# WangSimiao2000/MinecraftSkin_Raytracer

Measured on AMD Instinct MI355X. Metric: Mpixels/s, higher is better.
Workload: dtype f32; 1 GPU; 1920x1080, 4 bounces, 4 spp, 1 light, synthetic 64x64 skin (S64), pose 0, soft shadows 8, tile 32; parallelism=single GPU, frames_in_flight=4, hw_queues=4

## Files before the change

### include/mcrt.h

```cpp
#ifndef MCRT_H
#define MCRT_H

#include <stddef.h>
#include <stdint.h>

#ifdef __cplusplus
extern "C" {
#endif

#define MCRT_ABI_VERSION 3

#define MCRT_OK 0
#define MCRT_ERR_INVALID 1
#define MCRT_ERR_NO_DEVICE 2
#define MCRT_ERR_HIP 3
#define MCRT_ERR_NOMEM 4

typedef struct mcrt_config {
    int32_t width;
    int32_t height;
    int32_t max_bounces;
    int32_t samples_per_pixel;
    int32_t tile_size;
    int32_t thread_count;
// ... 308 lines not shown
int mcrt_build_skin_scene_model(const uint8_t* skin_rgba8, int skin_width, int skin_height, int model,
                                const float pose[12], mcrt_scene_desc** out);
int mcrt_scene_create_skin_model(int skin_height, int model, const float pose[12], const mcrt_scene_desc* look, int device, mcrt_scene** out);
int mcrt_skin_texel_model(int skin_height, int model, int mesh, int face_slot, int tx, int ty, int* skin_x, int* skin_y);
int mcrt_skin_pool_map_model(int skin_height, int model, int32_t* out, int capacity);
int mcrt_skin_view_table_model(int skin_height, int model, const float pose[12], const mcrt_scene_desc* look, void* out, size_t capacity);
int mcrt_skin_model_of(const uint8_t* skin_rgba8, int skin_width, int skin_height);
int mcrt_build_default_scene(const float pose[12], mcrt_scene_desc** out);
int mcrt_builtin_pose(int index, float pose_out[12]);
void mcrt_scene_desc_free(mcrt_scene_desc* desc);

size_t mcrt_scene_flatten(const mcrt_scene_desc* desc, void* blob, size_t capacity);

typedef struct mcrt_hit {
    int32_t hit;
    float t;
    float point[3];
    float normal[3];
    float texture_color[4];
    int32_t is_outer_layer;
} mcrt_hit;

int mcrt_probe_scene_blob(mcrt_scene* scene, void* out, size_t capacity);
int mcrt_probe_intersect(mcrt_scene* scene, const float* rays, int n, mcrt_hit* out);
int mcrt_probe_trace(mcrt_scene* scene, const mcrt_config* cfg, const float* rays, int n, int depth,
                     float* out_rgba);
int mcrt_probe_mt_uniform(int device, const uint32_t* seeds, int n_seeds, int n_draws, float* out);
int mcrt_probe_detmath(int device, int op, const float* x, const float* y, size_t n, float* out);
int mcrt_probe_detmath_range(int device, int op, uint32_t lo_bits, uint32_t hi_bits, float y0,
                             uint64_t* mismatches);
int mcrt_probe_div_const(int device, uint32_t d_first, uint32_t d_count, int mode, uint64_t* mismatches, uint32_t* a_failing_divisor);

#ifdef __cplusplus
}
#endif
#endif
```

### minecraftskin_raytracer_amd/_lib.py

```python
from __future__ import annotations

import ctypes as C
import os

from . import abi

PKG = os.path.dirname(os.path.abspath(__file__))
LIB_PATH = os.environ.get("MCRT_LIB") or os.path.join(PKG, "libmcrt.so")

_lib = None

EXPORTED_SYMBOLS = [
    "mcrt_config_init", "mcrt_generate_tiles", "mcrt_abi_version", "mcrt_device_count", "mcrt_last_error",
    "mcrt_render", "mcrt_render_tile", "mcrt_scene_create", "mcrt_scene_destroy", "mcrt_render_device", "mcrt_owned_pixel_rows",
    "mcrt_unpack_rows_device", "mcrt_quantize_rgba8_device", "mcrt_quantize_rgba8", "mcrt_last_timings",
    "mcrt_time_render_device", "mcrt_build_skin_scene", "mcrt_build_default_scene", "mcrt_builtin_pose",
    "mcrt_scene_desc_free", "mcrt_scene_flatten", "mcrt_probe_intersect", "mcrt_probe_trace",
    "mcrt_probe_mt_uniform", "mcrt_probe_detmath", "mcrt_probe_detmath_range", "mcrt_probe_div_const",
    "mcrt_render_device_ex", "mcrt_write_png_rgba8", "mcrt_encode_png_rgba8", "mcrt_write_png_f32", "mcrt_render_png",
    "mcrt_assemble_frame_device", "mcrt_scene_set_lanes", "mcrt_trim", "mcrt_scene_check", "mcrt_render_multi",
    "mcrt_render_rgba8", "mcrt_render_rect", "mcrt_render_batch_device", "mcrt_render_batch", "mcrt_last_batch_info",
    "mcrt_scene_set_background", "mcrt_render_ex", "mcrt_render_batch_ex", "mcrt_render_png_ex",
    "mcrt_bg_plate_info", "mcrt_draw_plate_info",
    "mcrt_render_layers_device", "mcrt_render_layers_batch_device", "mcrt_render_layers", "mcrt_render_layers_batch",
    "mcrt_scene_pick", "mcrt_skin_texel",
    "mcrt_render_ground_device", "mcrt_render_ground_batch_device", "mcrt_render_ground", "mcrt_scene_floor",
    "mcrt_render_reflection_device", "mcrt_render_reflection_batch_device", "mcrt_render_reflection",
    "mcrt_render_light_device", "mcrt_render_light_batch_device", "mcrt_render_light",
    "mcrt_scene_create_skin", "mcrt_scene_set_skin_device", "mcrt_scene_set_skins_batch_device", "mcrt_scene_set_skin",
    "mcrt_skin_pool_map", "mcrt_probe_scene_blob",
    "mcrt_bake_light_device", "mcrt_bake_light_batch_device", "mcrt_bake_light", "mcrt_bake_texel_table", "mcrt_scene_texels",
    "mcrt_scene_set_view", "mcrt_scene_set_view_device", "mcrt_scene_set_views_batch_device", "mcrt_skin_view_table",
    "mcrt_shot_init", "mcrt_shot_scratch_bytes", "mcrt_composite_shot_batch_device", "mcrt_render_shot_batch_device",
    "mcrt_render_shot_device", "mcrt_render_shot", "mcrt_render_shot_batch", "mcrt_render_shot_png",
    "mcrt_render_ground_occlusion_device", "mcrt_render_ground_occlusion_batch_device", "mcrt_render_ground_occlusion",
    "mcrt_shot_scratch_bytes_occ", "mcrt_render_shot_batch_device_occ", "mcrt_composite_shot_batch_device_occ",
    "mcrt_render_shot_batch_occ", "mcrt_render_shot_png_occ",
    "mcrt_shot_ex_init", "mcrt_shot_scratch_bytes_ex", "mcrt_composite_shot_batch_device_ex", "mcrt_render_shot_batch_device_ex",
    "mcrt_render_shot_batch_ex", "mcrt_render_shot_png_ex",
    "mcrt_build_skin_scene_model", "mcrt_scene_create_skin_model", "mcrt_skin_texel_model", "mcrt_skin_pool_map_model",
    "mcrt_skin_view_table_model", "mcrt_skin_model_of",
]


def load():
    global _lib
    if _lib is not None:
        return _lib
    if not os.path.exists(LIB_PATH):
        raise RuntimeError(
            f"{LIB_PATH} is missing: build it with `python -m minecraftskin_raytracer_amd.build` "
            "(hipcc --offload-arch=gfx950). There is no CPU fallback."
        )
# ... 141 lines not shown
```

### minecraftskin_raytracer_amd/api.py

```python
from __future__ import annotations

import ctypes as C
import os
from typing import Callable, List, Optional, Sequence, Tuple

import numpy as np

from . import abi
from ._lib import McrtError, check, load
from .abi import Config, Mesh, Scene, SceneDescHolder, Texture

Image = np.ndarray


def trim() -> None:
    load().mcrt_trim()


def device_count() -> int:
    return int(load().mcrt_device_count())


class _OwnedDescPtr(C.POINTER(abi.McrtSceneDesc)):

# ... 599 lines not shown
        self._skin_bytes()
        check(load().mcrt_scene_set_skin_device(self._h, C.c_void_p(ptr or None), C.c_void_p(stream)))

    def set_view(self, pose: Optional[Sequence[float]] = None, look=None) -> None:
        self._skin_bytes()
        p, d = _view_pose(pose), _as_desc(look) if look is not None else None
        check(load().mcrt_scene_set_view(self._h, abi.fptr(p) if p is not None else None, d.ptr if d is not None else None))

    def set_view_device(self, pose: Optional[Sequence[float]] = None, look=None, stream: int = 0) -> None:
        self._skin_bytes()
        p, d = _view_pose(pose), _as_desc(look) if look is not None else None
        check(load().mcrt_scene_set_view_device(self._h, abi.fptr(p) if p is not None else None, d.ptr if d is not None else None, C.c_void_p(stream)))

    def blob(self) -> bytes:
        lib = load()
        head = C.create_string_buffer(192)
        n = lib.mcrt_probe_scene_blob(self._h, head, 192)
        if n < 192:
            raise McrtError(n, lib.mcrt_last_error().decode("utf-8", "replace"))
        buf = C.create_string_buffer(n)
        if lib.mcrt_probe_scene_blob(self._h, buf, n) != n:
            raise McrtError(abi.MCRT_ERR_HIP, lib.mcrt_last_error().decode("utf-8", "replace"))
        return buf.raw

    def close(self):
        if self._h:
            load().mcrt_scene_destroy(self._h)
            self._h = C.c_void_p()

    def __del__(self):
        try:
            self.close()
        except Exception:
            pass

    def check(self) -> None:
        check(load().mcrt_scene_check(self._h))

    def set_lanes(self, lanes: int) -> None:
        check(load().mcrt_scene_set_lanes(self._h, int(lanes)))

    def set_background(self, mode: str) -> None:
        m = abi.background_mode(mode)
        check(load().mcrt_scene_set_background(self._h, m))

    def owned_pixel_rows(self, config: Config, first: int = 0, step: int = 1) -> int:
# ... 525 lines not shown
```

### minecraftskin_raytracer_amd/csrc/kernel_common.h

```cpp
#ifndef MCRT_KERNEL_COMMON_H
#define MCRT_KERNEL_COMMON_H

#include "kernels.h"
#include "rt_core.h"

#include <type_traits>

#ifdef MCRT_KERNEL_HOOKS
#include MCRT_KERNEL_HOOKS
#else
#define MCRT_HOOK_LIT_SHARED
#define MCRT_HOOK_LIT_CLASSIFIED(known, undecided, cand, O)
#define MCRT_HOOK_LIT_SHADED(lit, r)
#define MCRT_HOOK_RESOLVE_BEGIN()
#endif

namespace mcrt {

using namespace rt;

struct UDiv {
    unsigned d;
    int shift;
    __device__ __forceinline__ explicit UDiv(unsigned dv) : d(dv), shift((dv & (dv - 1u)) == 0u && dv != 0u ? static_cast<int>(__builtin_ctz(dv)) : -1) {}
    __device__ __forceinline__ unsigned div(unsigned n) const { return shift >= 0 ? n >> shift : n / d; }
};

struct TileGeom {
    int x, y, w, h;
    int owned_row;
    int frame_tile;
};

__device__ __forceinline__ uchar4 quantize_pixel(float4 c) {
    uchar4 q;
    q.x = static_cast<unsigned char>(sclamp(c.x, 0.0f, 1.0f) * 255.0f + 0.5f);
    q.y = static_cast<unsigned char>(sclamp(c.y, 0.0f, 1.0f) * 255.0f + 0.5f);
    q.z = static_cast<unsigned char>(sclamp(c.z, 0.0f, 1.0f) * 255.0f + 0.5f);
    q.w = static_cast<unsigned char>(sclamp(c.w, 0.0f, 1.0f) * 255.0f + 0.5f);
    return q;
}

__device__ __forceinline__ bool mesh_touches_tile(const FlatMesh& m, const TileGeom& t, const mcrt_config& cfg,
                                                  float aspect, float lens_pad) {
    float u0 = m.screen[0], v0 = m.screen[1], u1 = m.screen[2], v1 = m.screen[3];
    if (u0 > u1) return true;
    u0 -= lens_pad, v0 -= lens_pad, u1 += lens_pad, v1 += lens_pad;
    const float W = static_cast<float>(cfg.width), H = static_cast<float>(cfg.height);
    float tu0 = (2.0f * (static_cast<float>(t.x) - 2.0f) / W - 1.0f) * aspect - 1e-3f * aspect - 1e-3f;
    float tu1 = (2.0f * (static_cast<float>(t.x + t.w) + 2.0f) / W - 1.0f) * aspect + 1e-3f * aspect + 1e-3f;
    float tv1 = 1.0f - 2.0f * (static_cast<float>(t.y) - 2.0f) / H + 2e-3f;
    float tv0 = 1.0f - 2.0f * (static_cast<float>(t.y + t.h) + 2.0f) / H - 2e-3f;
    return !(u1 < tu0 || u0 > tu1 || v1 < tv0 || v0 > tv1);
}

struct LdsTables {
// ... 230 lines not shown
```

### minecraftskin_raytracer_amd/csrc/kernels.h

```cpp
#ifndef MCRT_KERNELS_H
#define MCRT_KERNELS_H

#include <hip/hip_runtime.h>
#include <stdint.h>

#include <vector>

#include "launch_shapes.h"
#include "mcrt.h"

namespace mcrt {

struct Shard {
    int first;
    int step;
    int tiles_x;
    int tiles_y;
    int owned_rows;
    int pack_first;
    int pack_step;
};

struct WaveSpace {
    float4* scol;
// ... 27 lines not shown
constexpr int kDivFrameMax = 16384;

constexpr uint32_t kSeedWindowHalf = 1u << 24;
constexpr uint32_t kSeedWindow = 1u << 25;

struct RenderParams {
    const uint8_t* scene;
    const uint32_t* seed_table;
    const uint32_t* seed_table_full;
    mcrt_config cfg;
    Shard shard;
    int layout;
    float* out;
    uint8_t* out8;
    uint32_t* tile_rng;
    const float4* bg_plate;
    const float* draw_plate;
    WaveSpace ws;
    int draws_per_sample;
    int stream_waves;
    int stream_parts;
    int stream_part_twists;
    int parts_per_tile;
    int lds_alpha_words;
    int lds_face_entries;
    int scene_in_lds;
    int scene_posed;
    int rows_per_batch;
    int bg_in_plan;
    int bg_kernel;
    int background;
    int lit_round;
    int lit_pass;
    int lit_lds_offset;
    int lit_lds_bytes;
    int flat;
    float inv_width, inv_height;
    int div_frame;
    int inside_fast;
    int bundle_decisions;
    int work_tickets;
    int shared_device;
    int grid_primary, grid_ao, grid_lit, grid_resolve;
    int rect_x, rect_y, rect_w, rect_h;
};

// ... 309 lines not shown
```

### minecraftskin_raytracer_amd/csrc/probes.cpp

```cpp
#include "host_internal.h"
#include "mcrt_detmath.h"

#include <cmath>
#include <thread>

using namespace mcrt;
using namespace mcrt_host;

namespace {
int finish_probe(hipError_t launched, void* out, const DeviceBuffer& d_out, size_t bytes, const char* what) {
    hipError_t e = launched;
    if (e == hipSuccess) e = hipMemcpy(out, d_out.ptr, bytes, hipMemcpyDeviceToHost);
    if (e != hipSuccess) return hip_fail(e, what);
    return MCRT_OK;
}
}

extern "C" {

int mcrt_probe_intersect(mcrt_scene* s, const float* rays, int n, mcrt_hit* out) {
    if (!s || !rays || !out || n < 0) return fail(MCRT_ERR_INVALID, "bad argument");
    if (n == 0) return MCRT_OK;
    HIP_TRY(hipSetDevice(s->device));
    DeviceBuffer d_rays, d_out;
    HIP_TRY(d_rays.reserve(static_cast<size_t>(n) * 24));
    HIP_TRY(d_out.reserve(static_cast<size_t>(n) * sizeof(mcrt_hit)));
    HIP_TRY(hipMemcpy(d_rays.ptr, rays, static_cast<size_t>(n) * 24, hipMemcpyHostToDevice));
    hipError_t e = launch_probe_intersect(static_cast<const uint8_t*>(s->blob.ptr), static_cast<float*>(d_rays.ptr), n,
                                          static_cast<mcrt_hit*>(d_out.ptr), nullptr);
    return finish_probe(e, out, d_out, static_cast<size_t>(n) * sizeof(mcrt_hit), "probe_intersect");
}

int mcrt_probe_scene_blob(mcrt_scene* s, void* out, size_t capacity) {
    if (!s || !out) return fail(MCRT_ERR_INVALID, "NULL argument");
    HIP_TRY(hipSetDevice(s->device));
    HIP_TRY(hipDeviceSynchronize());
    if (s->host_meshes.size() < sizeof(FlatHeader) || !s->blob.ptr) return fail(MCRT_ERR_INVALID, "the handle holds no scene");
    const size_t bytes = reinterpret_cast<const FlatHeader*>(s->host_meshes.data())->blob_bytes;
    HIP_TRY(hipMemcpy(out, s->blob.ptr, bytes < capacity ? bytes : capacity, hipMemcpyDeviceToHost));
    return static_cast<int>(bytes);
}

int mcrt_probe_trace(mcrt_scene* s, const mcrt_config* cfg, const float* rays, int n, int depth, float* out_rgba) {
    if (!s || !cfg || !rays || !out_rgba || n < 0) return fail(MCRT_ERR_INVALID, "bad argument");
    if (n == 0) return MCRT_OK;
    HIP_TRY(hipSetDevice(s->device));
    DeviceBuffer d_rays, d_out, d_rng, d_stack;
    HIP_TRY(d_rays.reserve(static_cast<size_t>(n) * 24));
    HIP_TRY(d_out.reserve(static_cast<size_t>(n) * 16));
    bool long_rng = (cfg->soft_shadows && 2 * cfg->shadow_samples > 227) || (cfg->ao_enabled && 2 * cfg->ao_samples > 227);
    if (long_rng) HIP_TRY(d_rng.reserve(static_cast<size_t>(n) * 624 * 4));
    if (cfg->max_bounces > 16) HIP_TRY(d_stack.reserve(static_cast<size_t>(n) * cfg->max_bounces * 16));
    HIP_TRY(hipMemcpy(d_rays.ptr, rays, static_cast<size_t>(n) * 24, hipMemcpyHostToDevice));
    hipError_t e = launch_probe_trace(static_cast<const uint8_t*>(s->blob.ptr), *cfg, static_cast<float*>(d_rays.ptr), n,
                                      depth, static_cast<float*>(d_out.ptr), static_cast<uint32_t*>(d_rng.ptr),
                                      static_cast<float*>(d_stack.ptr), nullptr);
    return finish_probe(e, out_rgba, d_out, static_cast<size_t>(n) * 16, "probe_trace");
}

int mcrt_probe_mt_uniform(int device, const uint32_t* seeds, int n_seeds, int n_draws, float* out) {
    if (!seeds || !out || n_seeds < 0 || n_draws < 0) return fail(MCRT_ERR_INVALID, "bad argument");
    if (n_seeds == 0 || n_draws == 0) return MCRT_OK;
    if (mcrt_device_count() <= 0) return fail(MCRT_ERR_NO_DEVICE, "no HIP device");
// ... 97 lines not shown
```

### minecraftskin_raytracer_amd/csrc/render_enqueue.cpp

```cpp
#include "host_internal.h"

#include <algorithm>
#include <cmath>
#include <cstring>

using namespace mcrt;
using namespace mcrt_host;

namespace {

thread_local int t_background_override = -1;
struct BackgroundOverride {
    explicit BackgroundOverride(int mode) { t_background_override = mode; }
    ~BackgroundOverride() { t_background_override = -1; }
    BackgroundOverride(const BackgroundOverride&) = delete;
    BackgroundOverride& operator=(const BackgroundOverride&) = delete;
};

int draws_per_sample(const mcrt_config& c) {
    int spp = c.samples_per_pixel > 1 ? c.samples_per_pixel : 1;
    return (spp > 1 ? 2 : 0) + ((c.dof_enabled && c.aperture > 1e-6f) ? 2 : 0);
}

int lane_count(const mcrt_scene* s, const mcrt_config& cfg, const Shard& sh) {
// ... 58 lines not shown
            for (int tx = tx0; tx <= tx1; ++tx) grid[static_cast<size_t>(ty) * sh.tiles_x + tx] = 1;
    }
    for (int j = 0; j < sh.owned_rows; ++j) {
        const int ty = sh.first + j * sh.step;
        int c = 0;
        for (int tx = 0; tx < sh.tiles_x; ++tx) c += grid[static_cast<size_t>(ty) * sh.tiles_x + tx];
        out[static_cast<size_t>(j)] = c;
    }
}

int prepare(mcrt_scene* sc, int li, int n_lanes, const mcrt_config* cfg, int first, int step, int layout, float* d_out,
            uint8_t* d_out8, RenderParams& p, std::vector<int>* row_touched_out = nullptr, const mcrt_tile* rect = nullptr) {
    Lane* s = &sc->lanes[li];
    std::memset(&p, 0, sizeof p);
    p.scene = static_cast<const uint8_t*>(sc->blob.ptr);
    p.seed_table = sc->seed_table;
    p.seed_table_full = sc->seed_table_full;
    static const bool decisions = !env_off("MCRT_BUNDLE_DECISIONS");
    p.bundle_decisions = decisions ? 1 : 0;
    static const bool inside_fast = !env_off("MCRT_INSIDE_FAST");
    p.inside_fast = inside_fast ? 1 : 0;
    static const bool work_tickets = !env_off("MCRT_WORK_TICKETS");
    p.work_tickets = work_tickets ? 1 : 0;
    p.cfg = *cfg;
    if (cfg->width > 0 && cfg->height > 0) {
        p.inv_width = 1.0f / static_cast<float>(cfg->width);
        p.inv_height = 1.0f / static_cast<float>(cfg->height);
        static const bool fast_div = !env_off("MCRT_DIV_FRAME");
        p.div_frame = (fast_div && cfg->width <= kDivFrameMax && cfg->height <= kDivFrameMax) ? 1 : 0;
    }
    p.shard = make_shard(*cfg, first + li * step, step * n_lanes);
    p.shard.pack_first = li;
    p.shard.pack_step = n_lanes;
    if (rect) {
        p.rect_x = rect->x, p.rect_y = rect->y, p.rect_w = rect->width, p.rect_h = rect->height;
        p.shard.first = 0, p.shard.step = 1, p.shard.tiles_x = 1, p.shard.tiles_y = 1, p.shard.owned_rows = 1;
        p.shard.pack_first = 0, p.shard.pack_step = 1;
    }
    p.layout = layout;
    p.out = d_out;
    p.out8 = d_out8;
    p.background = rect ? MCRT_BACKGROUND_REFERENCE : (t_background_override >= 0 ? t_background_override : sc->background);
    p.draws_per_sample = draws_per_sample(*cfg);
    const LdsFit fit = lds_fit(sc->alpha_words, sc->n_meshes, sc->posed);
    p.scene_in_lds = fit.view != kViewHbm ? 1 : 0;
    p.scene_posed = sc->posed ? 1 : 0;
// ... 1237 lines not shown
```

### minecraftskin_raytracer_amd/csrc/render_kernels.hip

```cpp
#include "kernel_common.h"

namespace mcrt {

using namespace rt;

struct FrameDiv {
    float w, h, rw, rh;
    bool fast;
    __device__ __forceinline__ explicit FrameDiv(const RenderParams& p)
        : w(static_cast<float>(p.cfg.width)), h(static_cast<float>(p.cfg.height)), rw(p.inv_width), rh(p.inv_height), fast(p.div_frame != 0) {}
    __device__ __forceinline__ float u(float x) const { return fast ? div_frame(x, w, rw) : x / w; }
    __device__ __forceinline__ float v(float y) const { return fast ? div_frame(y, h, rh) : y / h; }
};

__device__ __forceinline__ TileGeom tile_of(const RenderParams& p, int owned_tile) {
    TileGeom t;
    if (p.rect_w > 0) {
        t.x = p.rect_x, t.y = p.rect_y, t.w = p.rect_w, t.h = p.rect_h;
        t.owned_row = 0;
        t.frame_tile = 0;
        return t;
    }
    int k = owned_tile / p.shard.tiles_x;
    int tx = owned_tile - k * p.shard.tiles_x;
// ... 289 lines not shown
        const FlatMesh& m = sc.meshes[lane];
        float lens_pad = 0.0f;
        if (dof) {
            const float half_h = sc.hdr->cam_half_h, half_w = half_h * aspect;
            const float focus = cfg.focus_distance > 0.0f ? cfg.focus_distance : sc.hdr->cam_focus_auto;
            const float inv_f_lo = 1.0f / focus;
            const float inv_f_hi = __builtin_sqrtf(1.0f + half_w * half_w + half_h * half_h) / focus;
            const float inv_z_hi = 1.0f / m.depth[0], inv_z_lo = 1.0f / m.depth[1];
            const float d = fmaxf(fmaxf(fabsf(inv_z_hi - inv_f_lo), fabsf(inv_z_hi - inv_f_hi)),
                                  fmaxf(fabsf(inv_z_lo - inv_f_lo), fabsf(inv_z_lo - inv_f_hi)));
            lens_pad = cfg.aperture * d / half_h * 1.02f + 1e-3f;
            const float err = 4.0f * 1.1920929e-7f * (sc.hdr->mask_slack * (1.0f / kMaskSlack) + focus + cfg.aperture);
            const float r2 = half_w * half_w + half_h * half_h;
            const float rel = err * inv_f_hi * (1.0f + __builtin_sqrtf(r2));
            lens_pad += (2.0f * rel + err * inv_z_hi) / half_h;
            if (!(m.depth[0] > 0.0f) || !(focus > 0.0f) || !(lens_pad < 1e6f) || !(rel < 0.05f)) lens_pad = 1e30f;
        }
        touch = mesh_touches_tile(m, tg, cfg, aspect, lens_pad);
    }
    unsigned long long mask = __ballot(touch);
    if (!cull && sc.n_meshes > 0) mask = ~0ull;
    return mask;
}
__device__ __forceinline__ uint32_t plan_touched_tile(const RenderParams& p, const TileGeom& tg, int tile, unsigned long long mask) {
    const mcrt_config& cfg = p.cfg;
    const WaveSpace& ws = p.ws;
    ws.tile_mask[tile] = mask;
    if (mask == 0ull) return ~0u;
    const uint32_t spp = cfg.samples_per_pixel > 1 ? cfg.samples_per_pixel : 1;
    const uint32_t npix = static_cast<uint32_t>(tg.w) * static_cast<uint32_t>(tg.h);
    const uint32_t parts = static_cast<uint32_t>(p.parts_per_tile);
    const uint32_t per = (npix + parts - 1u) / parts;
    const uint32_t used = (npix + per - 1u) / per;
    const uint32_t ord = count_add(ws, kCntTiles, 1u);
    if (ord >= ws.tile_cap) {
        ws.counters[kCntOverflow] = 1u;
        ws.tile_mask[tile] = 0ull;
        return ~0u;
    }
    const uint32_t slot0 = count_add(ws, kCntUnits, used);
    const uint32_t base = ord * ws.tile_slots;
    for (uint32_t i = 0; i < used; ++i) {
        const uint32_t a = i * per, b = min(npix, a + per);
        ws.units[slot0 + i] = make_uint4(static_cast<uint32_t>(tile), a, b, base + a * spp);
    }
    return ord;
}

__device__ __forceinline__ void plan_tiles_body(const uint8_t* __restrict__ scene_blob, const uint32_t* __restrict__ tile_rng,
                                                float* __restrict__ tile_draws, float4* __restrict__ out_frame, uchar4* __restrict__ out8,
                                                const RenderParams& __restrict__ p, const int tile_base, const int n_tiles) {
    __shared__ __align__(16) uint32_t s_state[kStreamWaves][2 * 624];
    __shared__ uint32_t s_ord[kStreamWaves];
    const int wave = threadIdx.x >> 6, lane = threadIdx.x & 63;
    const int parts = p.stream_waves;
    const int per_wave = p.stream_parts / parts;
    const int slot = static_cast<int>(blockIdx.x) * kStreamWaves + wave;
    const int t = slot / parts, part = slot - t * parts;
    const bool valid = t < n_tiles;
    const int tile = tile_base + (valid ? t : 0);
    const TileGeom tg = tile_of(p, tile);
    const SceneView sc = view_of(scene_blob);
    const unsigned long long mask = valid ? tile_mesh_mask(sc, p, tg, lane) : 0ull;
    if (valid && part == 0 && lane == 0) s_ord[wave] = plan_touched_tile(p, tg, tile, mask);
    if (parts > 1) {
        __syncthreads();
    } else {
        __builtin_amdgcn_fence(__ATOMIC_SEQ_CST, "wavefront");
        __builtin_amdgcn_wave_barrier();
    }
    if (!valid) return;
    const uint32_t ord = s_ord[wave - part];
    const size_t stride = p.ws.draws_stride;
    const unsigned npix = static_cast<unsigned>(tg.w) * static_cast<unsigned>(tg.h);
    if (!p.bg_in_plan) {
        float4 unused;
        if (p.draws_per_sample > 0 && !(mask == 0ull && constant_background(sc, p, tg, unused)))
            tile_stream_wave(sc, tile_rng, tile_draws + static_cast<size_t>(t) * stride, nullptr, nullptr, p, tg, tile, part * per_wave, per_wave, s_state[wave], lane,
                             mask == 0ull && p.draws_per_sample == 4);
    } else if (mask != 0ull) {
        if (p.draws_per_sample > 0 && ord != ~0u && !p.draw_plate)
            tile_stream_wave(sc, tile_rng, tile_draws + static_cast<size_t>(ord) * stride, nullptr, nullptr, p, tg, tile, part * per_wave, per_wave, s_state[wave], lane);
    } else if (p.background == MCRT_BACKGROUND_TRANSPARENT) {
        fill_tile(p, tg, out_frame, out8, make_float4(0.0f, 0.0f, 0.0f, 0.0f), static_cast<unsigned>(part * 64 + lane), static_cast<unsigned>(parts) * 64u);
    } else if (float4 pixel; constant_background(sc, p, tg, pixel)) {
        fill_tile(p, tg, out_frame, out8, pixel, static_cast<unsigned>(part * 64 + lane), static_cast<unsigned>(parts) * 64u);
    } else if (p.cfg.samples_per_pixel > 1) {
// ... 100 lines not shown

    const SceneView scg = view_of(scene_blob);
    const mcrt_config& cfg = p.cfg;
    const WaveSpace& ws = p.ws;
    const uint32_t n_units = counted(ws, kCntUnits);
    if (blockIdx.x == 0 && threadIdx.x == 0) ws.frame_info[0] = n_units;
    if ((p.bg_in_plan || p.bg_kernel) && blockIdx.x >= n_units) return;
    const bool bounce_here = p.flat && cfg.max_bounces >= 1;
    const bool posed = kView != kViewLdsUnposed && p.scene_posed != 0;
    const typename ViewSel<kView>::type sc = ViewSel<kView>::make(scg, p, s_dyn);
    const int tid = threadIdx.x;
    const int spp = cfg.samples_per_pixel > 1 ? cfg.samples_per_pixel : 1;
    const int dd = p.draws_per_sample;
    const bool dof = cfg.dof_enabled && cfg.aperture > 1e-6f;
    const float aspect = static_cast<float>(cfg.width) / static_cast<float>(cfg.height);
    const FrameDiv fd(p);
    float focusDist = cfg.focus_distance;
    if (focusDist <= 0.0f) focusDist = sc.hdr->cam_focus_auto;
    const size_t stride = ws.draws_stride;

    uint32_t turn = 0;
    for (uint32_t u = blockIdx.x; u < n_units; u = next_work(p, kCntTicketPrimary, u, n_units, s_ticket, turn)) {
        const uint4 ud = ws.units[u];
        const int tile = static_cast<int>(ud.x);
        const unsigned pp0 = ud.y, pp1 = ud.z;
        const uint32_t slot_base = ud.w;
        const TileGeom tg = tile_of(p, tile);
        const unsigned long long mesh_mask = ws.tile_mask[tile];
        const float* draws = tile_draws + static_cast<size_t>(p.draw_plate ? static_cast<uint32_t>(tg.frame_tile)
                                                              : p.bg_in_plan ? slot_base / ws.tile_slots : static_cast<uint32_t>(tile - tile_base)) * stride;
        const unsigned n_samples = (pp1 - pp0) * static_cast<unsigned>(spp);

        uint32_t unit_hits = 0;
        for (unsigned s0 = 0; s0 < n_samples; s0 += kChunk) {
            bool is_hit = false;
            Ray ray{mk(0, 0, 0), mk(0, 0, 0)};
            Hit hit;
            hit.hit = false;
            uint32_t sample_slot = 0;
            const unsigned sidx = s0 + tid;
            if (sidx < n_samples) {
                const unsigned pix = pp0 + UDiv(static_cast<unsigned>(spp)).div(sidx);
                const unsigned uly = UDiv(static_cast<unsigned>(tg.w)).div(pix);
                const int ly = static_cast<int>(uly);
                const int lx = static_cast<int>(pix - uly * static_cast<unsigned>(tg.w));
                const int px = tg.x + lx, py = tg.y + ly;
                const float* jd = draws + (static_cast<size_t>(pp0) * spp + sidx) * dd;
                float jx = 0.5f, jy = 0.5f;
                int dpos = 0;
                if (spp > 1) {
                    jx = jd[0];
                    jy = jd[1];
                    dpos = 2;
                }
                const float su = fd.u(static_cast<float>(px) + jx);
                const float sv = fd.v(static_cast<float>(py) + jy);
                sample_slot = slot_base + sidx;
                ray = dof ? lens_ray(sc, su, sv, aspect, cfg.aperture, focusDist, jd[dpos], jd[dpos + 1])
                          : camera_ray(sc, su, sv, aspect);
                hit = hit_scene(sc, ray, mesh_mask);
                uint32_t code = kEndMiss;
                if (hit.hit && cfg.max_bounces < 0) {
                    const C4 col = background(sc, cfg, 0.5f, 0.5f);
                    ws.scol[sample_slot] = make_float4(col.r, col.g, col.b, col.a);
                    code = 0u;
                } else if (hit.hit) {
                    is_hit = true;
                    code = (p.flat && cfg.max_bounces == 0) ? 3u : 0u;
                }
                ws.end[sample_slot] = code;
// ... 753 lines not shown
        --dd;
    }
    for (; dd >= 0; --dd) {
        const float4 sd = lv[dd * plane];
        tail = fold_reflection(C4{sd.x, sd.y, sd.z, sd.w}, tail);
    }
    return make_float4(tail.r, tail.g, tail.b, tail.a);
}
template <bool kTransparent>
__device__ __forceinline__ void resolve_body(const uint8_t* __restrict__ scene_blob, const float* __restrict__ tile_draws,
                                             float4* __restrict__ out_frame, uchar4* __restrict__ out8, const RenderParams& __restrict__ p,
                                             const int tile_base) {
    __shared__ ResolveLds<kTransparent> s_lds;
    float4* s_col = s_lds.col;
    const WaveSpace& ws = p.ws;
    const mcrt_config& cfg = p.cfg;
    const SceneView scg = view_of(scene_blob);
    const FrameDiv fd(p);
    const uint32_t dd = static_cast<uint32_t>(p.draws_per_sample);
    auto unit_sample = [&](const uint4& d, const TileGeom& tg, const float* draws, uint32_t sidx, uint32_t spp_) __attribute__((always_inline)) -> float4 {
        const uint32_t slot = d.w + sidx;
        const uint32_t code = ws.end[slot];
        if (code != kEndMiss) return sample_colour(ws, slot, code, C4{scg.hdr->background[0], scg.hdr->background[1], scg.hdr->background[2], scg.hdr->background[3]});
        const unsigned pix = d.y + UDiv(spp_).div(sidx);
        const unsigned uly = UDiv(static_cast<unsigned>(tg.w)).div(pix);
        const int px = tg.x + static_cast<int>(pix - uly * static_cast<unsigned>(tg.w)), py = tg.y + static_cast<int>(uly);
        float jx = 0.5f, jy = 0.5f;
        if (spp_ > 1u) {
            const float2 j = *reinterpret_cast<const float2*>(draws + (static_cast<size_t>(d.y) * spp_ + sidx) * dd);
            jx = j.x, jy = j.y;
        }
        const C4 c = background(scg, cfg, fd.u(static_cast<float>(px) + jx), fd.v(static_cast<float>(py) + jy));
        return make_float4(c.r, c.g, c.b, c.a);
    };
    const uint32_t n_units = ws.frame_info[0];
    const uint32_t spp = cfg.samples_per_pixel > 1 ? static_cast<uint32_t>(cfg.samples_per_pixel) : 1u;
    const float inv_spp = 1.0f / static_cast<float>(spp);
    const uint32_t chunk_px = spp <= static_cast<uint32_t>(kBlock) ? static_cast<uint32_t>(kBlock) / spp : 0u;
    auto put_pixel = [&](const TileGeom& tg, uint32_t i, float4 acc) __attribute__((always_inline)) {
        const uint32_t uly = i / static_cast<uint32_t>(tg.w);
        const int ly = static_cast<int>(uly);
        const int lx = static_cast<int>(i - uly * static_cast<uint32_t>(tg.w));
        const int row = (p.layout == MCRT_LAYOUT_PACKED) ? ((p.shard.pack_first + tg.owned_row * p.shard.pack_step) * cfg.tile_size + ly) : (tg.y + ly);
        store_pixel(out_frame, out8, static_cast<size_t>(row) * cfg.width + (tg.x + lx),
                    make_float4(acc.x * inv_spp, acc.y * inv_spp, acc.z * inv_spp, acc.w * inv_spp));
    };
    auto hit_sample = [&](const uint4& d, uint32_t sidx, bool& hit) __attribute__((always_inline)) -> float4 {
        const uint32_t slot = d.w + sidx;
        const uint32_t code = ws.end[slot];
        hit = code != kEndMiss;
        if (!hit) return make_float4(0.0f, 0.0f, 0.0f, 0.0f);
        return sample_colour(ws, slot, code, C4{scg.hdr->background[0], scg.hdr->background[1], scg.hdr->background[2], scg.hdr->background[3]});
    };
    auto put_pixel_transparent = [&](const TileGeom& tg, uint32_t i, float4 acc, uint32_t n) __attribute__((always_inline)) {
        float4 v = make_float4(0.0f, 0.0f, 0.0f, 0.0f);
        if (n > 0u) {
            const float inv_n = 1.0f / static_cast<float>(n);
            v = make_float4(acc.x * inv_n, acc.y * inv_n, acc.z * inv_n, acc.w * inv_spp);
        }
        const uint32_t uly = i / static_cast<uint32_t>(tg.w);
        const int ly = static_cast<int>(uly);
        const int lx = static_cast<int>(i - uly * static_cast<uint32_t>(tg.w));
        const int row = (p.layout == MCRT_LAYOUT_PACKED) ? ((p.shard.pack_first + tg.owned_row * p.shard.pack_step) * cfg.tile_size + ly) : (tg.y + ly);
        store_pixel(out_frame, out8, static_cast<size_t>(row) * cfg.width + (tg.x + lx), v);
    };
    MCRT_HOOK_RESOLVE_BEGIN()
    if (blockIdx.x == 0) {
        for (int i = threadIdx.x; i < kCounterWords - 4; i += kBlock) ws.counter_base[i] = ws.counters[i];
    }
    for (uint32_t u = blockIdx.x; u < n_units; u += gridDim.x) {
        const uint4 d = ws.units[u];
        const TileGeom tg = tile_of(p, static_cast<int>(d.x));
        const uint32_t pp0 = d.y, pp1 = d.z;
        const float* draws = tile_draws + static_cast<size_t>(p.draw_plate ? static_cast<uint32_t>(tg.frame_tile)
                                                              : p.bg_in_plan ? d.w / ws.tile_slots : static_cast<uint32_t>(static_cast<int>(d.x) - tile_base)) * ws.draws_stride;
        if (chunk_px == 0u) {
            for (uint32_t i = pp0 + threadIdx.x; i < pp1; i += kBlock) {
                float4 acc = make_float4(0.0f, 0.0f, 0.0f, 0.0f);
                if constexpr (kTransparent) {
                    uint32_t n = 0;
                    for (uint32_t s = 0; s < spp; ++s) {
                        bool hit;
                        const float4 c = hit_sample(d, (i - pp0) * spp + s, hit);
                        if (!hit) continue;
                        acc.x += c.x, acc.y += c.y, acc.z += c.z, acc.w += c.w;
                        ++n;
                    }
                    put_pixel_transparent(tg, i, acc, n);
                } else {
                    for (uint32_t s = 0; s < spp; ++s) {
                        const float4 c = unit_sample(d, tg, draws, (i - pp0) * spp + s, spp);
                        acc.x += c.x, acc.y += c.y, acc.z += c.z, acc.w += c.w;
                    }
                    put_pixel(tg, i, acc);
                }
            }
            continue;
        }
        for (uint32_t p0 = pp0; p0 < pp1; p0 += chunk_px) {
            const uint32_t npx = min(chunk_px, pp1 - p0);
            if constexpr (kTransparent) {
                if (threadIdx.x < npx * spp) {
                    bool hit;
                    s_col[threadIdx.x] = hit_sample(d, (p0 - pp0) * spp + threadIdx.x, hit);
                    s_lds.hit[threadIdx.x] = hit ? 1 : 0;
                }
            } else {
                if (threadIdx.x < npx * spp) s_col[threadIdx.x] = unit_sample(d, tg, draws, (p0 - pp0) * spp + threadIdx.x, spp);
            }
            __syncthreads();
            if (threadIdx.x < npx) {
                float4 acc = make_float4(0.0f, 0.0f, 0.0f, 0.0f);
                if constexpr (kTransparent) {
                    uint32_t n = 0;
                    for (uint32_t s = 0; s < spp; ++s) {
                        if (!s_lds.hit[threadIdx.x * spp + s]) continue;
                        const float4 c = s_col[threadIdx.x * spp + s];
                        acc.x += c.x, acc.y += c.y, acc.z += c.z, acc.w += c.w;
                        ++n;
                    }
                    put_pixel_transparent(tg, p0 + threadIdx.x, acc, n);
                } else {
                    for (uint32_t s = 0; s < spp; ++s) {
                        const float4 c = s_col[threadIdx.x * spp + s];
                        acc.x += c.x, acc.y += c.y, acc.z += c.z, acc.w += c.w;
                    }
                    put_pixel(tg, p0 + threadIdx.x, acc);
                }
            }
            __syncthreads();
        }
    }
}
__global__ __launch_bounds__(kBlock) void resolve_kernel(const uint8_t* __restrict__ scene_blob, const float* __restrict__ tile_draws,
                                                         float4* __restrict__ out_frame, uchar4* __restrict__ out8, const RenderParams p,
                                                         const int tile_base) {
    resolve_body<false>(scene_blob, tile_draws, out_frame, out8, p, tile_base);
}
__global__ __launch_bounds__(kBlock) void resolve_transparent_kernel(const uint8_t* __restrict__ scene_blob, float4* __restrict__ out_frame,
                                                                     uchar4* __restrict__ out8, const RenderParams p, const int tile_base) {
    resolve_body<true>(scene_blob, nullptr, out_frame, out8, p, tile_base);
}

using ParamTable = const __attribute__((address_space(4))) RenderParams*;
__device__ __forceinline__ const RenderParams& frame_params(ParamTable table) { return *(const RenderParams*)(table + blockIdx.y); }
__global__ __launch_bounds__(64) void seed_tiles_batch_kernel(ParamTable table, int n_tiles) {
    seed_tiles_body(frame_params(table), n_tiles);
}
__global__ __launch_bounds__(64 * kStreamWaves) void advance_tiles_batch_kernel(ParamTable table, int n_tiles) {
    advance_tiles_body(frame_params(table), n_tiles);
// ... 168 lines not shown
```

### minecraftskin_raytracer_amd/csrc/render_plan.cpp

```cpp
#include "kernels.h"

#include "flat_scene.h"

#include <algorithm>
#include <cstdlib>
#include <cstring>

namespace mcrt {

using rt::kMtShortMax;

Shard make_shard(const mcrt_config& cfg, int first, int step) {
    Shard s{};
    s.first = first;
    s.step = step < 1 ? 1 : step;
    s.pack_first = 0;
    s.pack_step = 1;
    if (cfg.width <= 0 || cfg.height <= 0 || cfg.tile_size <= 0) return s;
    s.tiles_x = (cfg.width + cfg.tile_size - 1) / cfg.tile_size;
    s.tiles_y = (cfg.height + cfg.tile_size - 1) / cfg.tile_size;
    s.owned_rows = (first < s.tiles_y && first >= 0) ? (s.tiles_y - first + s.step - 1) / s.step : 0;
    return s;
}

static int int_knob(const char* name, int fallback) {
    const char* e = getenv(name);
    const int v = e ? atoi(e) : 0;
    return v > 0 ? v : fallback;
}

static bool needs_general_variant(const mcrt_config& c) {
    return (c.ao_enabled && (c.ao_samples <= 0 || 2 * c.ao_samples > kMtShortMax)) || (soft_sampling(c) && 2 * c.shadow_samples > kMtShortMax) ||
           c.max_bounces > kFlatMaxBounces;
}

static int choose_parts_per_tile(const RenderParams& p) {
    const mcrt_config& cfg = p.cfg;
    const long long spp = cfg.samples_per_pixel > 1 ? cfg.samples_per_pixel : 1;
    const long long tile_items = p.rect_w > 0 ? static_cast<long long>(p.rect_w) * p.rect_h * spp : static_cast<long long>(cfg.tile_size) * cfg.tile_size * spp;
    long long parts = (tile_items + kChunk - 1) / kChunk;
    const long long most = p.rect_w > 0 ? 4096 : 16;
    if (parts > most) parts = most;
    if (parts < 1) parts = 1;
    return static_cast<int>(parts);
}

WorkspaceBytes plan_workspace(RenderParams& p, size_t budget_bytes, const int* row_touched) {
    WorkspaceBytes w{};
    const mcrt_config& c = p.cfg;
    const int n_tiles = owned_tiles(p);
    p.parts_per_tile = choose_parts_per_tile(p);
    p.flat = needs_general_variant(c) ? 0 : 1;
    p.ws.stack_stride = c.max_bounces > 0 ? c.max_bounces + 1 : 1;
    const size_t spp = c.samples_per_pixel > 1 ? c.samples_per_pixel : 1;
    const size_t tile_w = p.rect_w > 0 ? static_cast<size_t>(p.rect_w) : static_cast<size_t>(c.tile_size < c.width ? c.tile_size : c.width);
    const size_t tile_h = p.rect_w > 0 ? static_cast<size_t>(p.rect_h) : static_cast<size_t>(c.tile_size < c.height ? c.tile_size : c.height);
    const size_t tile_slots = tile_w * tile_h * spp;
    const size_t S = soft_sampling(c) ? static_cast<size_t>(c.shadow_samples) : 0;
    const size_t A = c.ao_enabled && c.ao_samples > 0 ? static_cast<size_t>(c.ao_samples) : 0;
    const size_t rays = S > A ? S : A;
    const size_t recs = p.flat ? static_cast<size_t>(1 + (c.max_bounces > 0 ? c.max_bounces : 0)) : 2;
    const size_t hbm_rays = p.flat ? 0 : rays;
    const size_t ray_recs = p.flat ? 1 : recs;
    const size_t per_entry = 16 + 4 + recs * (5 * 16 + 4) + ray_recs * (12 * hbm_rays + (hbm_rays ? 8 : 0) + 4) + 4 + 16 * static_cast<size_t>(p.ws.stack_stride);
    {
        const size_t pairs = S ? S : 1;
        size_t pass = kLitLdsBytes / (12 * pairs);
// ... 308 lines not shown
```

Measured before the change: 19450 Mpixels/s.

## Split tiles into compact 2D pixel blocks instead of row-range units

Work units inside a tile can now be rectangular sub-blocks (chosen near-square, fitting one chunk) instead of contiguous row ranges. Compact blocks should make rays within a unit more coherent, which helps cache reuse and cuts divergence in traversal. Unit emission in the planner is also spread across wave lanes instead of lane 0 only. The cost is an extra pixel mapping (a divide plus an offset) per sample and a new unit encoding that the primary and resolve kernels must share. A probe API for inspecting unit records is added as well.

```diff
diff --git a/include/mcrt.h b/include/mcrt.h
--- a/include/mcrt.h
+++ b/include/mcrt.h
@@ -354,6 +354,7 @@
 } mcrt_hit;
 
 int mcrt_probe_scene_blob(mcrt_scene* scene, void* out, size_t capacity);
+int mcrt_probe_units(mcrt_scene* scene, uint32_t* records, uint32_t* hits, int capacity);
 int mcrt_probe_intersect(mcrt_scene* scene, const float* rays, int n, mcrt_hit* out);
 int mcrt_probe_trace(mcrt_scene* scene, const mcrt_config* cfg, const float* rays, int n, int depth,
                      float* out_rgba);
diff --git a/minecraftskin_raytracer_amd/_lib.py b/minecraftskin_raytracer_amd/_lib.py
--- a/minecraftskin_raytracer_amd/_lib.py
+++ b/minecraftskin_raytracer_amd/_lib.py
@@ -28,7 +28,7 @@
     "mcrt_render_reflection_device", "mcrt_render_reflection_batch_device", "mcrt_render_reflection",
     "mcrt_render_light_device", "mcrt_render_light_batch_device", "mcrt_render_light",
     "mcrt_scene_create_skin", "mcrt_scene_set_skin_device", "mcrt_scene_set_skins_batch_device", "mcrt_scene_set_skin",
-    "mcrt_skin_pool_map", "mcrt_probe_scene_blob",
+    "mcrt_skin_pool_map", "mcrt_probe_scene_blob", "mcrt_probe_units",
     "mcrt_bake_light_device", "mcrt_bake_light_batch_device", "mcrt_bake_light", "mcrt_bake_texel_table", "mcrt_scene_texels",
     "mcrt_scene_set_view", "mcrt_scene_set_view_device", "mcrt_scene_set_views_batch_device", "mcrt_skin_view_table",
     "mcrt_shot_init", "mcrt_shot_scratch_bytes", "mcrt_composite_shot_batch_device", "mcrt_render_shot_batch_device",
diff --git a/minecraftskin_raytracer_amd/api.py b/minecraftskin_raytracer_amd/api.py
--- a/minecraftskin_raytracer_amd/api.py
+++ b/minecraftskin_raytracer_amd/api.py
@@ -645,6 +645,17 @@
         if lib.mcrt_probe_scene_blob(self._h, buf, n) != n:
             raise McrtError(abi.MCRT_ERR_HIP, lib.mcrt_last_error().decode("utf-8", "replace"))
         return buf.raw
+
+    def units(self) -> dict:
+        fn = load().mcrt_probe_units
+        fn.restype, fn.argtypes = C.c_int, [C.c_void_p, C.c_void_p, C.c_void_p, C.c_int]
+        n = fn(self._h, None, None, 0)
+        if n < 0:
+            raise McrtError(n, load().mcrt_last_error().decode("utf-8", "replace"))
+        rec, hits = np.zeros((n, 4), np.uint32), np.zeros(n, np.uint32)
+        if n and fn(self._h, rec.ctypes.data, hits.ctypes.data, n) != n:
+            raise McrtError(abi.MCRT_ERR_HIP, load().mcrt_last_error().decode("utf-8", "replace"))
+        return {"records": rec, "hits": hits}
 
     def close(self):
         if self._h:
diff --git a/minecraftskin_raytracer_amd/csrc/kernel_common.h b/minecraftskin_raytracer_amd/csrc/kernel_common.h
--- a/minecraftskin_raytracer_amd/csrc/kernel_common.h
+++ b/minecraftskin_raytracer_amd/csrc/kernel_common.h
@@ -32,6 +32,28 @@
     int frame_tile;
 };
 
+constexpr uint32_t kUnitBlock = 1u << 31;
+__device__ __forceinline__ int unit_tile(const uint4& ud) { return static_cast<int>(ud.x & ~kUnitBlock); }
+__device__ __forceinline__ uint32_t unit_pixels(const uint4& ud) { return (ud.x & kUnitBlock) ? (ud.z & 0xffffu) * (ud.z >> 16) : ud.z - ud.y; }
+struct UnitMap {
+    uint32_t koff, x0, y0;
+    UDiv by_w;
+    __device__ __forceinline__ UnitMap(const uint4& ud, const TileGeom& tg)
+        : koff((ud.x & kUnitBlock) ? 0u : ud.y), x0((ud.x & kUnitBlock) ? (ud.y & 0xffffu) : 0u), y0((ud.x & kUnitBlock) ? (ud.y >> 16) : 0u),
+          by_w((ud.x & kUnitBlock) ? (ud.z & 0xffffu) : static_cast<uint32_t>(tg.w)) {}
+    __device__ __forceinline__ void rel(uint32_t k, uint32_t& col, uint32_t& row) const {
+        const uint32_t q = k + koff;
+        row = by_w.div(q);
+        col = q - row * by_w.d;
+    }
+    __device__ __forceinline__ void pixel(uint32_t k, int& lx, int& ly) const {
+        uint32_t col, row;
+        rel(k, col, row);
+        lx = static_cast<int>(x0 + col);
+        ly = static_cast<int>(y0 + row);
+    }
+};
+__device__ __forceinline__ void unit_pixel(const uint4& ud, const TileGeom& tg, uint32_t k, int& lx, int& ly) { UnitMap(ud, tg).pixel(k, lx, ly); }
 __device__ __forceinline__ uchar4 quantize_pixel(float4 c) {
     uchar4 q;
     q.x = static_cast<unsigned char>(sclamp(c.x, 0.0f, 1.0f) * 255.0f + 0.5f);
diff --git a/minecraftskin_raytracer_amd/csrc/kernels.h b/minecraftskin_raytracer_amd/csrc/kernels.h
--- a/minecraftskin_raytracer_amd/csrc/kernels.h
+++ b/minecraftskin_raytracer_amd/csrc/kernels.h
@@ -73,6 +73,8 @@
     int stream_parts;
     int stream_part_twists;
     int parts_per_tile;
+    int unit_blocks;
+    int unit_gx, unit_gy, unit_bw, unit_bh;
     int lds_alpha_words;
     int lds_face_entries;
     int scene_in_lds;
diff --git a/minecraftskin_raytracer_amd/csrc/probes.cpp b/minecraftskin_raytracer_amd/csrc/probes.cpp
--- a/minecraftskin_raytracer_amd/csrc/probes.cpp
+++ b/minecraftskin_raytracer_amd/csrc/probes.cpp
@@ -39,6 +39,21 @@
     const size_t bytes = reinterpret_cast<const FlatHeader*>(s->host_meshes.data())->blob_bytes;
     HIP_TRY(hipMemcpy(out, s->blob.ptr, bytes < capacity ? bytes : capacity, hipMemcpyDeviceToHost));
     return static_cast<int>(bytes);
+}
+
+int mcrt_probe_units(mcrt_scene* s, uint32_t* records, uint32_t* hits, int capacity) {
+    if (!s || capacity < 0) return fail(MCRT_ERR_INVALID, "bad argument");
+    HIP_TRY(hipSetDevice(s->device));
+    HIP_TRY(hipDeviceSynchronize());
+    const Lane& ln = s->lanes[0];
+    if (!ln.counters.ptr || !ln.units.ptr || !ln.unit_hits.ptr) return 0;
+    uint32_t n_units = 0;
+    HIP_TRY(hipMemcpy(&n_units, static_cast<const uint32_t*>(ln.counters.ptr) + 2 * kCounterWords, 4, hipMemcpyDeviceToHost));
+    if (n_units > 0x7fffffffu || static_cast<size_t>(n_units) * 16 > ln.units.bytes) return fail(MCRT_ERR_INVALID, "the lane's unit count does not fit its workspace");
+    const size_t n = n_units < static_cast<uint32_t>(capacity) ? n_units : static_cast<size_t>(capacity);
+    if (records && n) HIP_TRY(hipMemcpy(records, ln.units.ptr, n * 16, hipMemcpyDeviceToHost));
+    if (hits && n) HIP_TRY(hipMemcpy(hits, ln.unit_hits.ptr, n * 4, hipMemcpyDeviceToHost));
+    return static_cast<int>(n_units);
 }
 
 int mcrt_probe_trace(mcrt_scene* s, const mcrt_config* cfg, const float* rays, int n, int depth, float* out_rgba) {
diff --git a/minecraftskin_raytracer_amd/csrc/render_enqueue.cpp b/minecraftskin_raytracer_amd/csrc/render_enqueue.cpp
--- a/minecraftskin_raytracer_amd/csrc/render_enqueue.cpp
+++ b/minecraftskin_raytracer_amd/csrc/render_enqueue.cpp
@@ -104,6 +104,8 @@
     p.inside_fast = inside_fast ? 1 : 0;
     static const bool work_tickets = !env_off("MCRT_WORK_TICKETS");
     p.work_tickets = work_tickets ? 1 : 0;
+    static const bool unit_blocks = !env_off("MCRT_UNIT_BLOCKS");
+    p.unit_blocks = (unit_blocks && !rect) ? 1 : 0;
     p.cfg = *cfg;
     if (cfg->width > 0 && cfg->height > 0) {
         p.inv_width = 1.0f / static_cast<float>(cfg->width);
diff --git a/minecraftskin_raytracer_amd/csrc/render_kernels.hip b/minecraftskin_raytracer_amd/csrc/render_kernels.hip
--- a/minecraftskin_raytracer_amd/csrc/render_kernels.hip
+++ b/minecraftskin_raytracer_amd/csrc/render_kernels.hip
@@ -335,27 +335,54 @@
     if (!cull && sc.n_meshes > 0) mask = ~0ull;
     return mask;
 }
-__device__ __forceinline__ uint32_t plan_touched_tile(const RenderParams& p, const TileGeom& tg, int tile, unsigned long long mask) {
-    const mcrt_config& cfg = p.cfg;
-    const WaveSpace& ws = p.ws;
-    ws.tile_mask[tile] = mask;
-    if (mask == 0ull) return ~0u;
-    const uint32_t spp = cfg.samples_per_pixel > 1 ? cfg.samples_per_pixel : 1;
+__device__ __forceinline__ uint32_t tile_unit_count(const RenderParams& p, const TileGeom& tg) {
+    if (p.unit_blocks)
+        return static_cast<uint32_t>((tg.w + p.unit_bw - 1) / p.unit_bw) * static_cast<uint32_t>((tg.h + p.unit_bh - 1) / p.unit_bh);
     const uint32_t npix = static_cast<uint32_t>(tg.w) * static_cast<uint32_t>(tg.h);
     const uint32_t parts = static_cast<uint32_t>(p.parts_per_tile);
     const uint32_t per = (npix + parts - 1u) / parts;
-    const uint32_t used = (npix + per - 1u) / per;
-    const uint32_t ord = count_add(ws, kCntTiles, 1u);
-    if (ord >= ws.tile_cap) {
-        ws.counters[kCntOverflow] = 1u;
-        ws.tile_mask[tile] = 0ull;
-        return ~0u;
-    }
-    const uint32_t slot0 = count_add(ws, kCntUnits, used);
+    return (npix + per - 1u) / per;
+}
+__device__ __forceinline__ uint4 tile_unit(const RenderParams& p, const TileGeom& tg, uint32_t i) {
+    if (p.unit_blocks) {
+        const uint32_t cols = static_cast<uint32_t>((tg.w + p.unit_bw - 1) / p.unit_bw);
+        const uint32_t by = i / cols, bx = i - by * cols;
+        const uint32_t x0 = bx * static_cast<uint32_t>(p.unit_bw), y0 = by * static_cast<uint32_t>(p.unit_bh);
+        const uint32_t w = min(static_cast<uint32_t>(p.unit_bw), static_cast<uint32_t>(tg.w) - x0);
+        const uint32_t h = min(static_cast<uint32_t>(p.unit_bh), static_cast<uint32_t>(tg.h) - y0);
+        return make_uint4(kUnitBlock, x0 | (y0 << 16), w | (h << 16), y0 * static_cast<uint32_t>(tg.w) + h * x0);
+    }
+    const uint32_t npix = static_cast<uint32_t>(tg.w) * static_cast<uint32_t>(tg.h);
+    const uint32_t parts = static_cast<uint32_t>(p.parts_per_tile);
+    const uint32_t per = (npix + parts - 1u) / parts;
+    const uint32_t a = i * per;
+    return make_uint4(0u, a, min(npix, a + per), a);
+}
+__device__ __forceinline__ uint32_t plan_touched_tile(const RenderParams& p, const TileGeom& tg, int tile, unsigned long long mask, int lane) {
+    const mcrt_config& cfg = p.cfg;
+    const WaveSpace& ws = p.ws;
+    if (lane == 0) ws.tile_mask[tile] = mask;
+    if (mask == 0ull) return ~0u;
+    const uint32_t spp = cfg.samples_per_pixel > 1 ? cfg.samples_per_pixel : 1;
+    const uint32_t used = tile_unit_count(p, tg);
+    uint32_t ord = 0, slot0 = 0;
+    if (lane == 0) {
+        ord = count_add(ws, kCntTiles, 1u);
+        if (ord >= ws.tile_cap) {
+            ws.counters[kCntOverflow] = 1u;
+            ws.tile_mask[tile] = 0ull;
+            ord = ~0u;
+        } else {
+            slot0 = count_add(ws, kCntUnits, used);
+        }
+    }
+    ord = static_cast<uint32_t>(__shfl(static_cast<int>(ord), 0));
+    slot0 = static_cast<uint32_t>(__shfl(static_cast<int>(slot0), 0));
+    if (ord == ~0u) return ~0u;
     const uint32_t base = ord * ws.tile_slots;
-    for (uint32_t i = 0; i < used; ++i) {
-        const uint32_t a = i * per, b = min(npix, a + per);
-        ws.units[slot0 + i] = make_uint4(static_cast<uint32_t>(tile), a, b, base + a * spp);
+    for (uint32_t i = static_cast<uint32_t>(lane); i < used; i += 64u) {
+        const uint4 u = tile_unit(p, tg, i);
+        ws.units[slot0 + i] = make_uint4(static_cast<uint32_t>(tile) | u.x, u.y, u.z, base + u.w * spp);
     }
     return ord;
 }
@@ -375,7 +402,10 @@
     const TileGeom tg = tile_of(p, tile);
     const SceneView sc = view_of(scene_blob);
     const unsigned long long mask = valid ? tile_mesh_mask(sc, p, tg, lane) : 0ull;
-    if (valid && part == 0 && lane == 0) s_ord[wave] = plan_touched_tile(p, tg, tile, mask);
+    if (valid && part == 0) {
+        const uint32_t planned = plan_touched_tile(p, tg, tile, mask, lane);
+        if (lane == 0) s_ord[wave] = planned;
+    }
     if (parts > 1) {
         __syncthreads();
     } else {
@@ -522,14 +552,17 @@
     uint32_t turn = 0;
     for (uint32_t u = blockIdx.x; u < n_units; u = next_work(p, kCntTicketPrimary, u, n_units, s_ticket, turn)) {
         const uint4 ud = ws.units[u];
-        const int tile = static_cast<int>(ud.x);
-        const unsigned pp0 = ud.y, pp1 = ud.z;
+        const int tile = unit_tile(ud);
         const uint32_t slot_base = ud.w;
+        const unsigned n_samples = unit_pixels(ud) * static_cast<unsigned>(spp);
         const TileGeom tg = tile_of(p, tile);
         const unsigned long long mesh_mask = ws.tile_mask[tile];
         const float* draws = tile_draws + static_cast<size_t>(p.draw_plate ? static_cast<uint32_t>(tg.frame_tile)
                                                               : p.bg_in_plan ? slot_base / ws.tile_slots : static_cast<uint32_t>(tile - tile_base)) * stride;
-        const unsigned n_samples = (pp1 - pp0) * static_cast<unsigned>(spp);
+        const UnitMap um(ud, tg);
+        const int px0 = tg.x + static_cast<int>(um.x0), py0 = tg.y + static_cast<int>(um.y0);
+        const unsigned tile_w = static_cast<unsigned>(tg.w);
+        const float* unit_draws = draws + static_cast<size_t>(um.y0 * tile_w + um.x0) * spp * dd;
 
         uint32_t unit_hits = 0;
         for (unsigned s0 = 0; s0 < n_samples; s0 += kChunk) {
@@ -540,12 +573,11 @@
             uint32_t sample_slot = 0;
             const unsigned sidx = s0 + tid;
             if (sidx < n_samples) {
-                const unsigned pix = pp0 + UDiv(static_cast<unsigned>(spp)).div(sidx);
-                const unsigned uly = UDiv(static_cast<unsigned>(tg.w)).div(pix);
-                const int ly = static_cast<int>(uly);
-                const int lx = static_cast<int>(pix - uly * static_cast<unsigned>(tg.w));
-                const int px = tg.x + lx, py = tg.y + ly;
-                const float* jd = draws + (static_cast<size_t>(pp0) * spp + sidx) * dd;
+                const unsigned k = UDiv(static_cast<unsigned>(spp)).div(sidx);
+                unsigned col, row;
+                um.rel(k, col, row);
+                const int px = px0 + static_cast<int>(col), py = py0 + static_cast<int>(row);
+                const float* jd = unit_draws + (static_cast<size_t>(row * tile_w + col - k) * spp + sidx) * dd;
                 float jx = 0.5f, jy = 0.5f;
                 int dpos = 0;
                 if (spp > 1) {
@@ -1345,12 +1377,13 @@
         const uint32_t slot = d.w + sidx;
         const uint32_t code = ws.end[slot];
         if (code != kEndMiss) return sample_colour(ws, slot, code, C4{scg.hdr->background[0], scg.hdr->background[1], scg.hdr->background[2], scg.hdr->background[3]});
-        const unsigned pix = d.y + UDiv(spp_).div(sidx);
-        const unsigned uly = UDiv(static_cast<unsigned>(tg.w)).div(pix);
-        const int px = tg.x + static_cast<int>(pix - uly * static_cast<unsigned>(tg.w)), py = tg.y + static_cast<int>(uly);
+        const uint32_t k = UDiv(spp_).div(sidx);
+        int lx, ly;
+        unit_pixel(d, tg, k, lx, ly);
+        const int px = tg.x + lx, py = tg.y + ly;
         float jx = 0.5f, jy = 0.5f;
         if (spp_ > 1u) {
-            const float2 j = *reinterpret_cast<const float2*>(draws + (static_cast<size_t>(d.y) * spp_ + sidx) * dd);
+            const float2 j = *reinterpret_cast<const float2*>(draws + (static_cast<size_t>(ly * tg.w + lx) * spp_ + (sidx - k * spp_)) * dd);
             jx = j.x, jy = j.y;
         }
         const C4 c = background(scg, cfg, fd.u(static_cast<float>(px) + jx), fd.v(static_cast<float>(py) + jy));
@@ -1360,10 +1393,9 @@
     const uint32_t spp = cfg.samples_per_pixel > 1 ? static_cast<uint32_t>(cfg.samples_per_pixel) : 1u;
     const float inv_spp = 1.0f / static_cast<float>(spp);
     const uint32_t chunk_px = spp <= static_cast<uint32_t>(kBlock) ? static_cast<uint32_t>(kBlock) / spp : 0u;
-    auto put_pixel = [&](const TileGeom& tg, uint32_t i, float4 acc) __attribute__((always_inline)) {
-        const uint32_t uly = i / static_cast<uint32_t>(tg.w);
-        const int ly = static_cast<int>(uly);
-        const int lx = static_cast<int>(i - uly * static_cast<uint32_t>(tg.w));
+    auto put_pixel = [&](const uint4& d, const TileGeom& tg, uint32_t k, float4 acc) __attribute__((always_inline)) {
+        int lx, ly;
+        unit_pixel(d, tg, k, lx, ly);
         const int row = (p.layout == MCRT_LAYOUT_PACKED) ? ((p.shard.pack_first + tg.owned_row * p.shard.pack_step) * cfg.tile_size + ly) : (tg.y + ly);
         store_pixel(out_frame, out8, static_cast<size_t>(row) * cfg.width + (tg.x + lx),
                     make_float4(acc.x * inv_spp, acc.y * inv_spp, acc.z * inv_spp, acc.w * inv_spp));
@@ -1375,15 +1407,14 @@
         if (!hit) return make_float4(0.0f, 0.0f, 0.0f, 0.0f);
         return sample_colour(ws, slot, code, C4{scg.hdr->background[0], scg.hdr->background[1], scg.hdr->background[2], scg.hdr->background[3]});
     };
-    auto put_pixel_transparent = [&](const TileGeom& tg, uint32_t i, float4 acc, uint32_t n) __attribute__((always_inline)) {
+    auto put_pixel_transparent = [&](const uint4& d, const TileGeom& tg, uint32_t k, float4 acc, uint32_t n) __attribute__((always_inline)) {
         float4 v = make_float4(0.0f, 0.0f, 0.0f, 0.0f);
         if (n > 0u) {
             const float inv_n = 1.0f / static_cast<float>(n);
             v = make_float4(acc.x * inv_n, acc.y * inv_n, acc.z * inv_n, acc.w * inv_spp);
         }
-        const uint32_t uly = i / static_cast<uint32_t>(tg.w);
-        const int ly = static_cast<int>(uly);
-        const int lx = static_cast<int>(i - uly * static_cast<uint32_t>(tg.w));
+        int lx, ly;
+        unit_pixel(d, tg, k, lx, ly);
         const int row = (p.layout == MCRT_LAYOUT_PACKED) ? ((p.shard.pack_first + tg.owned_row * p.shard.pack_step) * cfg.tile_size + ly) : (tg.y + ly);
         store_pixel(out_frame, out8, static_cast<size_t>(row) * cfg.width + (tg.x + lx), v);
     };
@@ -1393,10 +1424,11 @@
     }
     for (uint32_t u = blockIdx.x; u < n_units; u += gridDim.x) {
         const uint4 d = ws.units[u];
-        const TileGeom tg = tile_of(p, static_cast<int>(d.x));
-        const uint32_t pp0 = d.y, pp1 = d.z;
+        const int tile = unit_tile(d);
+        const TileGeom tg = tile_of(p, tile);
+        const uint32_t pp0 = 0u, pp1 = unit_pixels(d);
         const float* draws = tile_draws + static_cast<size_t>(p.draw_plate ? static_cast<uint32_t>(tg.frame_tile)
-                                                              : p.bg_in_plan ? d.w / ws.tile_slots : static_cast<uint32_t>(static_cast<int>(d.x) - tile_base)) * ws.draws_stride;
+                                                              : p.bg_in_plan ? d.w / ws.tile_slots : static_cast<uint32_t>(tile - tile_base)) * ws.draws_stride;
         if (chunk_px == 0u) {
             for (uint32_t i = pp0 + threadIdx.x; i < pp1; i += kBlock) {
                 float4 acc = make_float4(0.0f, 0.0f, 0.0f, 0.0f);
@@ -1409,13 +1441,13 @@
                         acc.x += c.x, acc.y += c.y, acc.z += c.z, acc.w += c.w;
                         ++n;
                     }
-                    put_pixel_transparent(tg, i, acc, n);
+                    put_pixel_transparent(d, tg, i, acc, n);
                 } else {
                     for (uint32_t s = 0; s < spp; ++s) {
                         const float4 c = unit_sample(d, tg, draws, (i - pp0) * spp + s, spp);
                         acc.x += c.x, acc.y += c.y, acc.z += c.z, acc.w += c.w;
                     }
-                    put_pixel(tg, i, acc);
+                    put_pixel(d, tg, i, acc);
                 }
             }
             continue;
@@ -1442,13 +1474,13 @@
                         acc.x += c.x, acc.y += c.y, acc.z += c.z, acc.w += c.w;
                         ++n;
                     }
-                    put_pixel_transparent(tg, p0 + threadIdx.x, acc, n);
+                    put_pixel_transparent(d, tg, p0 + threadIdx.x, acc, n);
                 } else {
                     for (uint32_t s = 0; s < spp; ++s) {
                         const float4 c = s_col[threadIdx.x * spp + s];
                         acc.x += c.x, acc.y += c.y, acc.z += c.z, acc.w += c.w;
                     }
-                    put_pixel(tg, p0 + threadIdx.x, acc);
+                    put_pixel(d, tg, p0 + threadIdx.x, acc);
                 }
             }
             __syncthreads();
diff --git a/minecraftskin_raytracer_amd/csrc/render_plan.cpp b/minecraftskin_raytracer_amd/csrc/render_plan.cpp
--- a/minecraftskin_raytracer_amd/csrc/render_plan.cpp
+++ b/minecraftskin_raytracer_amd/csrc/render_plan.cpp
@@ -34,7 +34,7 @@
            c.max_bounces > kFlatMaxBounces;
 }
 
-static int choose_parts_per_tile(const RenderParams& p) {
+static int choose_parts_per_tile(RenderParams& p) {
     const mcrt_config& cfg = p.cfg;
     const long long spp = cfg.samples_per_pixel > 1 ? cfg.samples_per_pixel : 1;
     const long long tile_items = p.rect_w > 0 ? static_cast<long long>(p.rect_w) * p.rect_h * spp : static_cast<long long>(cfg.tile_size) * cfg.tile_size * spp;
@@ -42,7 +42,27 @@
     const long long most = p.rect_w > 0 ? 4096 : 16;
     if (parts > most) parts = most;
     if (parts < 1) parts = 1;
-    return static_cast<int>(parts);
+    p.unit_gx = p.unit_gy = p.unit_bw = p.unit_bh = 0;
+    if (p.rect_w > 0 || cfg.tile_size <= 0 || cfg.tile_size > 0xffff) p.unit_blocks = 0;
+    if (!p.unit_blocks) return static_cast<int>(parts);
+    const long long T = cfg.tile_size;
+    long long best_key = -1;
+    for (long long gx = 1; gx <= 16; ++gx)
+        for (long long gy = 1; gx * gy <= 16; ++gy) {
+            const long long bw = (T + gx - 1) / gx, bh = (T + gy - 1) / gy;
+            const long long lo = bw < bh ? bw : bh, hi = bw < bh ? bh : bw;
+            if (bw * bh * spp > kChunk || hi > 2 * lo) continue;
+            const long long key = ((gx * gy) << 40) | ((hi - lo) << 8) | (bw >= bh ? 0 : 1);
+            if (best_key < 0 || key < best_key) {
+                best_key = key;
+                p.unit_gx = static_cast<int>(gx), p.unit_gy = static_cast<int>(gy), p.unit_bw = static_cast<int>(bw), p.unit_bh = static_cast<int>(bh);
+            }
+        }
+    if (best_key < 0) {
+        p.unit_blocks = 0;
+        return static_cast<int>(parts);
+    }
+    return p.unit_gx * p.unit_gy;
 }
 
 WorkspaceBytes plan_workspace(RenderParams& p, size_t budget_bytes, const int* row_touched) {
```

After: 20600 Mpixels/s, median of 6. +5.9%, better.
